# Tarseus/eam-rl4co

Measured on AMD Instinct MI355X. Metric: env-steps/sec (batch x num_loc / s), AttentionModel construction rollout, higher is better.
Workload: dtype f32; 1 GPU; TSP num_loc=100 batch=1024/GPU AM greedy rollout (encoder + cache + decode loop + reward); global_batch=1024, launch=hipGraph replay

## Files before the change

eam_rl4co_amd/csrc/encoder_fused.hip:

```cpp
#include "encoder_fused.hpp"

namespace eamrl {

constexpr int SA = 140;
constexpr int GA = 34;
constexpr int SQ = 66;

struct ALayout {
    float* HB;
    static constexpr int S = SA;
    __device__ float* col(int c) const { return HB + (c & 3) * GA + (c >> 2); }
    __device__ void store4(int row, int q4, float4 v) const
    {
        float* p = HB + row * SA + q4;
        p[0] = v.x; p[GA] = v.y; p[2 * GA] = v.z; p[3 * GA] = v.w;
    }
    __device__ float4 load4(int row, int q4) const
    {
        const float* p = HB + row * SA + q4;
        return make_float4(p[0], p[GA], p[2 * GA], p[3 * GA]);
    }
    __device__ void mirror(int, int, float) const {}
};

#ifdef EAMRL_STAMPS
__device__ unsigned long long g_enc_stamps[24];
#define ESTAMP(i) do { const unsigned long long now_ = __builtin_readcyclecounter(); st_acc[i] += now_ - st_t; st_t = now_; } while (0)
#else
#define ESTAMP(i) do { } while (0)
#endif

__device__ __forceinline__ f32x4 mfma4(float a, float b, f32x4 c) { return __builtin_amdgcn_mfma_f32_16x16x4f32(a, b, c, 0, 0, 0); }

typedef float f32x2v __attribute__((ext_vector_type(2)));
__device__ __forceinline__ float2 lds_read_b64(const float* p)
{
    typedef const volatile __attribute__((address_space(3))) f32x2v* lds_ptr;
    const f32x2v v = *(lds_ptr)(p);
    return make_float2(v.x, v.y);
}

__device__ __forceinline__ float4 global_load_b128(const float* p)
{
    typedef const __attribute__((address_space(1))) f32x4* global_ptr;
    const f32x4 v = *(global_ptr)(p);
    return make_float4(v[0], v[1], v[2], v[3]);
}

template <int CT>
__device__ __forceinline__ void load_b0(float4 (&b0)[CT], const float* const (&wp)[CT])
{
#pragma unroll
    for (int ct = 0; ct < CT; ++ct) b0[ct] = global_load_b128(wp[ct]);
}

template <int RTW, int S>
__device__ __forceinline__ void load_a0(float2 (&a0)[RTW][2], const float* arow, int nrt)
{
#pragma unroll
    for (int rt = 0; rt < RTW; ++rt)
        if (rt < nrt) {
            a0[rt][0] = lds_read_b64(arow + rt * 16 * S);
            a0[rt][1] = lds_read_b64(arow + rt * 16 * S + 2);
        }
}

template <int RTW, int CT, int S, bool SWAP, int NRT, int NU>
__device__ __forceinline__ void gemm_pass_n(f32x4 (&acc)[RTW][CT], const float* arow, const float* const (&wp)[CT],
                                            const float4 (&b0)[CT], const float2 (&a0)[RTW][2])
{
    float4 b[2][CT];
    float2 a[2][NRT][2];
#pragma unroll
    for (int ct = 0; ct < CT; ++ct) b[0][ct] = b0[ct];
#pragma unroll
    for (int rt = 0; rt < NRT; ++rt) { a[0][rt][0] = a0[rt][0]; a[0][rt][1] = a0[rt][1]; }
#pragma unroll
    for (int u = 0; u < NU; ++u) {
        const int c = u & 1, n = c ^ 1;
        __builtin_amdgcn_sched_barrier(0);
        if (u + 1 < NU) {
#pragma unroll
            for (int ct = 0; ct < CT; ++ct) b[n][ct] = global_load_b128(wp[ct] + (u + 1) * 256);
#pragma unroll
            for (int rt = 0; rt < NRT; ++rt) {
                a[n][rt][0] = lds_read_b64(arow + rt * 16 * S + 4 * (u + 1));
                a[n][rt][1] = lds_read_b64(arow + rt * 16 * S + 4 * (u + 1) + 2);
            }
        }
#pragma unroll
        for (int rt = 0; rt < NRT; ++rt) {
#pragma unroll
            for (int ct = 0; ct < CT; ++ct)
                acc[rt][ct] = SWAP ? mfma4(b[c][ct].x, a[c][rt][0].x, acc[rt][ct]) : mfma4(a[c][rt][0].x, b[c][ct].x, acc[rt][ct]);
#pragma unroll
            for (int ct = 0; ct < CT; ++ct)
                acc[rt][ct] = SWAP ? mfma4(b[c][ct].y, a[c][rt][0].y, acc[rt][ct]) : mfma4(a[c][rt][0].y, b[c][ct].y, acc[rt][ct]);
#pragma unroll
            for (int ct = 0; ct < CT; ++ct)
                acc[rt][ct] = SWAP ? mfma4(b[c][ct].z, a[c][rt][1].x, acc[rt][ct]) : mfma4(a[c][rt][1].x, b[c][ct].z, acc[rt][ct]);
#pragma unroll
            for (int ct = 0; ct < CT; ++ct)
                acc[rt][ct] = SWAP ? mfma4(b[c][ct].w, a[c][rt][1].y, acc[rt][ct]) : mfma4(a[c][rt][1].y, b[c][ct].w, acc[rt][ct]);
        }
        if (u + 1 < NU) {
            __builtin_amdgcn_sched_group_barrier(0x20, CT, 0);
#pragma unroll
            for (int i = 0; i < 2 * NRT; ++i) {
                __builtin_amdgcn_sched_group_barrier(0x8, 2, 0);
                __builtin_amdgcn_sched_group_barrier(0x100, 1, 0);
            }
            __builtin_amdgcn_sched_group_barrier(0x8, 4 * NRT * (CT - 1), 0);
        }
    }
    __builtin_amdgcn_sched_barrier(0);
}

template <int RTW, int CT, int S, int NU, bool SWAP = false, int NLOW = RTW>
__device__ __forceinline__ void gemm_pass(f32x4 (&acc)[RTW][CT], const float* arow, int nrt, const float* const (&wp)[CT],
                                          const float4 (&b0)[CT], const float2 (&a0)[RTW][2])
{
    if (NLOW == RTW || nrt == RTW) gemm_pass_n<RTW, CT, S, SWAP, RTW, NU>(acc, arow, wp, b0, a0);
    else gemm_pass_n<RTW, CT, S, SWAP, NLOW, NU>(acc, arow, wp, b0, a0);
}

template <int RTW>
__device__ __forceinline__ void residual_norm_store(const f32x4 (&acc)[RTW][2], float* HB, int row0, int nrt, int cw, int j, int G,
                                                    int norm, const float* cst )
{
    asm volatile("" : "+v"(j), "+v"(G));
#pragma unroll
    for (int ct = 0; ct < 2; ++ct) {
        const int c = 32 * cw + 16 * ct + j;
        const float sc = cst[c], sh = cst[FE + c];
        float* col = HB + (c & 3) * GA + (c >> 2);
#pragma unroll
        for (int rt = 0; rt < RTW; ++rt)
            if (rt < nrt) {
#pragma unroll
                for (int r = 0; r < 4; ++r) {
                    float* p = col + (row0 + 16 * rt + 4 * G + r) * SA;
                    float v = *p + acc[rt][ct][r];
                    if (norm == EAMRL_NORM_BATCH_EVAL) v = fma_(v, sc, sh);
                    *p = v;
                }
            }
    }
}

template <int RTT>
__global__ __launch_bounds__(512, 2) void k_encoder_fused(FusedArgs a)
{
    constexpr int RTA = (RTT + 1) / 2;
    constexpr int RTW = RTA;
    constexpr int ROWS = 16 * RTT;
    constexpr int SV = ROWS + 4;
    extern __shared__ __attribute__((aligned(16))) float lds[];
    float* HB = lds;
    float* QA = HB + ROWS * SA;
    float* KB = QA + ROWS * SQ;
    float* VT = KB + ROWS * SQ;
    float* HID = QA;
    float* CST = VT + 64 * SV;
    static_assert(ROWS * SA <= 2 * ROWS * SQ + 64 * SV, "HID must fit QA | KB | VT");
    const ALayout L{HB};

    const int tid = threadIdx.x, lane = tid & 63;
    const int wv = __builtin_amdgcn_readfirstlane(tid >> 6);
    const int cw = wv & 3, rw = wv >> 2;
    const int j = lane & 15, G = lane >> 4;
    const int M = a.M;
    const int row0 = rw ? 16 * RTA : 0;
    const int nrt = rw ? RTT - RTA : RTA;
    const int64_t inst = blockIdx.x;
    const float* hrow = HB + (row0 + j) * SA + G * GA;
#ifdef EAMRL_STAMPS
    unsigned long long st_acc[20] = {0, 0, 0, 0, 0, 0, 0, 0, 0, 0, 0, 0, 0, 0, 0, 0, 0, 0, 0, 0}, st_t = __builtin_readcyclecounter();
#endif

    if (a.h_in) load_h<ROWS>(a.h_in, M, L);
    else init_embedding<ROWS>(a.init, M, L);
    __syncthreads();
    ESTAMP(0);

    for (int layer = 0; layer < a.nlayers; ++layer) {
        const eamrl_encoder_layer& Ly = a.L[layer];
        const float* wp1[3];
        float4 b1[3];
        float2 a1[RTW][2];
#pragma unroll
        for (int x = 0; x < 3; ++x) wp1[x] = Ly.Wqkv + ((int64_t)(8 * x + cw) * (FE / 16)) * 256 + lane * 4;
        load_b0<3>(b1, wp1);
        load_a0<RTW, SA>(a1, hrow, nrt);
        for (int i = tid; i < NCST; i += blockDim.x) {
            float v;
            if (i < C_BO) v = Ly.bqkv[i];
            else if (i < C_B1) v = Ly.bo[i - C_BO];
            else if (i < C_B2) v = Ly.b1[i - C_B1];
            else if (i < C_N1) v = Ly.b2[i - C_B2];
            else {
                const bool second = i >= C_N2;
                const int k = (i - (second ? C_N2 : C_N1));
                const int c = k & (FE - 1);
                const float* gam = second ? Ly.n2_gamma : Ly.n1_gamma;
                const float* bet = second ? Ly.n2_beta : Ly.n1_beta;
                if (a.norm == EAMRL_NORM_BATCH_EVAL) {
                    const float* mean = second ? Ly.n2_mean : Ly.n1_mean;
                    const float* var = second ? Ly.n2_var : Ly.n1_var;
                    const float sc = gam[c] / __builtin_sqrtf(var[c] + a.eps);
                    const float ms = mean[c] * sc;
                    v = k < FE ? sc : bet[c] - ms;
                } else {
                    v = k < FE ? gam[c] : bet[c];
                }
            }
            CST[i] = v;
        }
        __syncthreads();
        f32x4 acc_o[RTW][2];
#pragma unroll
        for (int ct = 0; ct < 2; ++ct) {
            const float b = CST[C_BO + 32 * cw + 16 * ct + j];
#pragma unroll
            for (int rt = 0; rt < RTW; ++rt) acc_o[rt][ct] = splat4(b);
        }
        for (int hg = 0; hg < 2; ++hg) {
            const float* wp3[2];
            float4 b3[2];
#pragma unroll
            for (int ct = 0; ct < 2; ++ct)
                wp3[ct] = Ly.Wo + ((int64_t)(2 * cw + ct) * (FE / 16) + 4 * hg) * 256 + lane * 4;
            {
                f32x4 acc[RTW][3];
                const int ctq = 4 * hg + cw;
#pragma unroll
                for (int x = 0; x < 3; ++x) {
                    const float b = CST[C_BQKV + 16 * (8 * x + ctq) + j];
#pragma unroll
                    for (int rt = 0; rt < RTW; ++rt) acc[rt][x] = splat4(b);
                }
                ESTAMP(16);
                gemm_pass<RTW, 3, SA, FE / 16, false, RTT - RTA>(acc, hrow, nrt, wp1, b1, a1);
                ESTAMP(17);
                load_b0<2>(b3, wp3);
                int je = j, Ge = G;
                asm volatile("" : "+v"(je), "+v"(Ge));
                float* qcol = QA + (je & 3) * 16 + 4 * cw + (je >> 2);
                float* kcol = KB + (je & 3) * 16 + 4 * cw + (je >> 2);
                float* vrow = VT + (16 * cw + je) * SV;
#pragma unroll
                for (int rt = 0; rt < RTW; ++rt)
                    if (rt < nrt) {
                        const int rbase = row0 + 16 * rt + 4 * Ge;
#pragma unroll
                        for (int r = 0; r < 4; ++r) {
                            qcol[(rbase + r) * SQ] = acc[rt][0][r] * 0.25f;
                            kcol[(rbase + r) * SQ] = acc[rt][1][r];
                        }
                        *reinterpret_cast<float4*>(vrow + rbase) =
                            make_float4(acc[rt][2][0], acc[rt][2][1], acc[rt][2][2], acc[rt][2][3]);
                    }
            }
            ESTAMP(1);
            __syncthreads();
            ESTAMP(2);
            {
                int jp = j, Gp = G;
                asm volatile("" : "+v"(jp), "+v"(Gp));
                const int pi = 4 * (jp & 3) + (jp >> 2);
                float kf[RTT][4];
#pragma unroll
                for (int kt = 0; kt < RTT; ++kt) {
                    const float* p = KB + (16 * kt + pi) * SQ + Gp * 16 + 4 * cw;
                    const float2 lo = *reinterpret_cast<const float2*>(p), hi = *reinterpret_cast<const float2*>(p + 2);
                    kf[kt][0] = lo.x; kf[kt][1] = lo.y; kf[kt][2] = hi.x; kf[kt][3] = hi.y;
                }
                float vf[4 * RTT];
                const int NT = (M + 3) >> 2;
                constexpr int FULLT = RTT == 7 ? 4 : RTT == 4 ? 2 : 0;
#pragma unroll
                for (int t = 0; t < 4 * RTT; ++t) vf[t] = (t < NT) ? VT[(16 * cw + jp) * SV + 4 * t + Gp] : 0.0f;
                for (int q = 0; q < nrt; ++q) {
                    const int qrow = row0 + 16 * q + jp;
                    const float* qp = QA + qrow * SQ + Gp * 16 + 4 * cw;
                    const float2 qlo = *reinterpret_cast<const float2*>(qp), qhi = *reinterpret_cast<const float2*>(qp + 2);
                    f32x4 s[RTT];
                    float m = -INFINITY;
#pragma unroll
                    for (int kt = 0; kt < RTT; ++kt) s[kt] = mfma4(kf[kt][0], qlo.x, splat4(0.0f));
#pragma unroll
                    for (int kt = 0; kt < RTT; ++kt) s[kt] = mfma4(kf[kt][1], qlo.y, s[kt]);
#pragma unroll
                    for (int kt = 0; kt < RTT; ++kt) s[kt] = mfma4(kf[kt][2], qhi.x, s[kt]);
#pragma unroll
                    for (int kt = 0; kt < RTT; ++kt) s[kt] = mfma4(kf[kt][3], qhi.y, s[kt]);
#pragma unroll
                    for (int kt = 0; kt < RTT; ++kt) {
                        if (kt >= FULLT && 16 * kt + 16 > M) {
#pragma unroll
                            for (int r = 0; r < 4; ++r)
                                if (16 * kt + 4 * r + Gp >= M) s[kt][r] = -INFINITY;
                        }
                        m = vmax5_raw(m, s[kt][0], s[kt][1], s[kt][2], s[kt][3]);
                    }
                    {
                        auto r16 = __builtin_amdgcn_permlane16_swap(__float_as_uint(m), __float_as_uint(m), false, false);
                        m = vmax_raw(__uint_as_float(r16[0]), __uint_as_float(r16[1]));
                        auto r32 = __builtin_amdgcn_permlane32_swap(__float_as_uint(m), __float_as_uint(m), false, false);
                        m = vmax_raw(__uint_as_float(r32[0]), __uint_as_float(r32[1]));
                    }
#pragma unroll
                    for (int kt = 0; kt < RTT; ++kt) {
                        f32x2 e01 = (f32x2){s[kt][0], s[kt][1]} - splat2(m), e23 = (f32x2){s[kt][2], s[kt][3]} - splat2(m);
                        d_expf2_nonpos_x2(e01, e23);
                        s[kt] = (f32x4){e01.x, e01.y, e23.x, e23.y};
                    }
                    float zp = s[0][0];
#pragma unroll
                    for (int t = 1; t < 4 * RTT; ++t) zp = zp + s[t >> 2][t & 3];
                    {
                        auto r16 = __builtin_amdgcn_permlane16_swap(__float_as_uint(zp), __float_as_uint(zp), false, false);
                        zp = __uint_as_float(r16[0]) + __uint_as_float(r16[1]);
                        auto r32 = __builtin_amdgcn_permlane32_swap(__float_as_uint(zp), __float_as_uint(zp), false, false);
                        zp = __uint_as_float(r32[0]) + __uint_as_float(r32[1]);
                    }
                    f32x4 o = splat4(0.0f);
#pragma unroll
                    for (int kt = 0; kt < RTT; ++kt)
                        if (kt < FULLT || 16 * kt < M) {
#pragma unroll
                            for (int r = 0; r < 4; ++r) o = mfma4(vf[4 * kt + r], s[kt][r], o);
                        }
                    float* op = QA + qrow * SQ + 4 * cw + Gp;
#pragma unroll
                    for (int r = 0; r < 4; ++r) op[r * 16] = o[r] / zp;
                }
            }
            ESTAMP(3);
            __syncthreads();
            ESTAMP(4);
            float2 a3[RTW][2];
            load_a0<RTW, SQ>(a3, QA + (row0 + j) * SQ + G * 16, nrt);
            if (hg == 0) {
#pragma unroll
                for (int x = 0; x < 3; ++x) wp1[x] += 4 * (FE / 16) * 256;
                load_b0<3>(b1, wp1);
                load_a0<RTW, SA>(a1, hrow, nrt);
            }
            gemm_pass<RTW, 2, SQ, 4, false, RTT - RTA>(acc_o, QA + (row0 + j) * SQ + G * 16, nrt, wp3, b3, a3);
            ESTAMP(5);
            __syncthreads();
            ESTAMP(6);
        }
        const float* wp4[2];
        float4 b4[2];
        float2 a4[RTW][2];
#pragma unroll
        for (int ct = 0; ct < 2; ++ct) wp4[ct] = Ly.W1 + ((int64_t)(2 * cw + ct) * (FE / 16)) * 256 + lane * 4;
        load_b0<2>(b4, wp4);
        residual_norm_store<RTW>(acc_o, HB, row0, nrt, cw, j, G, a.norm, CST + C_N1);
        __syncthreads();
        if (a.norm == EAMRL_NORM_INSTANCE) {
            instance_norm(L, M, a.eps, CST + C_N1);
            __syncthreads();
        }
        load_a0<RTW, SA>(a4, hrow, nrt);
        ESTAMP(7);
        f32x4 acc_f[RTW][2];
#pragma unroll
        for (int ct = 0; ct < 2; ++ct) {
            const float b = CST[C_B2 + 32 * cw + 16 * ct + j];
#pragma unroll
            for (int rt = 0; rt < RTW; ++rt) acc_f[rt][ct] = splat4(b);
        }
        for (int ch = 0; ch < FF / 128; ++ch) {
            const float* wp5[2];
            float4 b5[2];
#pragma unroll
            for (int ct = 0; ct < 2; ++ct)
                wp5[ct] = Ly.W2 + ((int64_t)(2 * cw + ct) * (FF / 16) + 8 * ch) * 256 + lane * 4;
            {
                f32x4 acc[RTW][2];
#pragma unroll
                for (int ct = 0; ct < 2; ++ct) {
                    const float b = CST[C_B1 + 16 * (8 * ch + 2 * cw + ct) + j];
#pragma unroll
                    for (int rt = 0; rt < RTW; ++rt) acc[rt][ct] = splat4(b);
                }
                ESTAMP(14);
                gemm_pass<RTW, 2, SA, FE / 16, false, RTT - RTA>(acc, hrow, nrt, wp4, b4, a4);
                ESTAMP(15);
                load_b0<2>(b5, wp5);
#pragma unroll
                for (int ct = 0; ct < 2; ++ct) {
                    const int c = 32 * cw + 16 * ct + j;
                    float* col = HID + (c & 3) * GA + (c >> 2);
#pragma unroll
                    for (int rt = 0; rt < RTW; ++rt)
                        if (rt < nrt) {
#pragma unroll
                            for (int r = 0; r < 4; ++r) {
                                const float v = acc[rt][ct][r];
                                col[(row0 + 16 * rt + 4 * G + r) * SA] = !(v > 0.0f) ? 0.0f : v;
                            }
                        }
                }
            }
            ESTAMP(8);
            __syncthreads();
            ESTAMP(9);
            float2 a5[RTW][2];
            load_a0<RTW, SA>(a5, HID + (row0 + j) * SA + G * GA, nrt);
            if (ch + 1 < FF / 128) {
#pragma unroll
                for (int ct = 0; ct < 2; ++ct) wp4[ct] += 8 * (FE / 16) * 256;
                load_b0<2>(b4, wp4);
                load_a0<RTW, SA>(a4, hrow, nrt);
            }
            gemm_pass<RTW, 2, SA, 8, false, RTT - RTA>(acc_f, HID + (row0 + j) * SA + G * GA, nrt, wp5, b5, a5);
            ESTAMP(10);
            __syncthreads();
            ESTAMP(11);
        }
        residual_norm_store<RTW>(acc_f, HB, row0, nrt, cw, j, G, a.norm, CST + C_N2);
        __syncthreads();
        if (a.norm == EAMRL_NORM_INSTANCE) {
            instance_norm(L, M, a.eps, CST + C_N2);
            __syncthreads();
        }
        ESTAMP(12);
    }
    if (a.h_out) store_h(a.h_out, M, L);
    ESTAMP(13);
    if (a.cache.gctx) graph_context(a.cache.Wg, a.cache.gctx, M, L, CST);
    if (a.cache.out) {
        float* STG = QA;
        float* crow = a.cache.out + (inst * (int64_t)M) * a.cache.ld;
        for (int sl = 0; sl <= a.cache.nproj; ++sl) {
            const bool lp = sl == a.cache.nproj;
            f32x4 acc[RTW][2];
            const float* wp[2];
            float4 b0[2];
#pragma unroll
            for (int ct = 0; ct < 2; ++ct)
                wp[ct] = (lp ? a.cache.WoutT : a.cache.Wc + (int64_t)sl * FE * FE) + ((int64_t)(2 * cw + ct) * (FE / 16)) * 256 + lane * 4;
            load_b0<2>(b0, wp);
#pragma unroll
            for (int ct = 0; ct < 2; ++ct)
#pragma unroll
                for (int rt = 0; rt < RTW; ++rt) acc[rt][ct] = splat4(0.0f);
            if (lp) __syncthreads();
            const float* arow = (lp ? STG : HB) + (row0 + j) * SA + G * GA;
            float2 a0[RTW][2];
            load_a0<RTW, SA>(a0, arow, nrt);
            gemm_pass<RTW, 2, SA, FE / 16, true, RTT - RTA>(acc, arow, nrt, wp, b0, a0);
#pragma unroll
            for (int rt = 0; rt < RTW; ++rt)
                if (rt < nrt) {
                    const int node = row0 + 16 * rt + j;
#pragma unroll
                    for (int ct = 0; ct < 2; ++ct) {
                        const int c = 32 * cw + 16 * ct + 4 * G;
                        const f32x4 v = acc[rt][ct];
                        if (node < M)
                            *reinterpret_cast<float4*>(crow + (int64_t)node * a.cache.ld + sl * FE + c) = make_float4(v[0], v[1], v[2], v[3]);
                        if (sl == 2) {
                            float* p = STG + node * SA + (c >> 2);
                            p[0] = v[0]; p[GA] = v[1]; p[2 * GA] = v[2]; p[3 * GA] = v[3];
                        }
                    }
                }
        }
    }
#ifdef EAMRL_STAMPS
    if (lane == 0) {
        for (int i = 0; i < 20; ++i) atomicAdd(&g_enc_stamps[i], st_acc[i]);
        atomicAdd(&g_enc_stamps[20], 1ull);
    }
#endif
}

__global__ void k_pack_mfma_b(const float* __restrict__ W, float* __restrict__ Wp, int N, int K)
{
    const int64_t idx = (int64_t)blockIdx.x * blockDim.x + threadIdx.x;
    if (idx >= (int64_t)N * K) return;
    const int q = (int)(idx & 3), l = (int)((idx >> 2) & 63);
    const int64_t blk = idx >> 8;
    const int u = (int)(blk % (K / 16)), ct = (int)(blk / (K / 16));
    const int j = l & 15, g = l >> 4;
    Wp[idx] = W[(int64_t)(16 * ct + j) * K + 16 * u + 4 * q + g];
}

int launch_pack_mfma_b(const float* W, float* Wp, int N, int K, hipStream_t st)
{
    const int64_t n = (int64_t)N * K;
    hipLaunchKernelGGL(k_pack_mfma_b, dim3((unsigned)((n + 255) / 256)), dim3(256), 0, st, W, Wp, N, K);
    return hipGetLastError() == hipSuccess ? 0 : EAMRL_E_LAUNCH;
}

#ifdef EAMRL_STAMPS
extern "C" __attribute__((visibility("default"))) int eamrl_debug_read_enc_stamps(unsigned long long* out, int reset)
{
    if (hipMemcpyFromSymbol(out, HIP_SYMBOL(g_enc_stamps), sizeof(g_enc_stamps)) != hipSuccess) return -1;
    if (reset) {
        unsigned long long z[24] = {0};
        if (hipMemcpyToSymbol(HIP_SYMBOL(g_enc_stamps), z, sizeof(z)) != hipSuccess) return -1;
    }
    return 0;
}
#endif

bool encoder_fused_supports(int M, int E, int H, int FFdim, int nlayers)
{
    return M >= 1 && M <= 112 && E == FE && H == FH && FFdim == FF && nlayers >= 1 && nlayers <= MAX_FUSED_LAYERS;
}

int launch_encoder_fused(const float* h_in, float* h_out, int64_t B, int M, int nlayers, int norm, float eps,
                         const eamrl_encoder_layer* layers, const eamrl_encoder_cache* cache, const eamrl_encoder_init* init,
                         int dtype, hipStream_t st)
{
    if (B <= 0) return 0;
    FusedArgs a = {};
    a.h_in = init ? nullptr : h_in; a.h_out = h_out; a.M = M; a.nlayers = nlayers; a.norm = norm; a.eps = eps;
    if (cache) {
        a.cache = *cache;
        if (!cache->Wg || !cache->gctx) a.cache.Wg = a.cache.gctx = nullptr;
    }
    if (init) a.init = *init;
    for (int l = 0; l < nlayers; ++l) a.L[l] = layers[l];
    if (dtype != DTYPE_F32) return launch_encoder_fused16(a, B, dtype, st);
    return launch_fused(a, B, st, [](auto rtt) {
        constexpr int RTT = decltype(rtt)::value, ROWS = 16 * RTT;
        return FusedVariant{k_encoder_fused<RTT>, ((size_t)ROWS * SA + 2 * (size_t)ROWS * SQ + 64 * (size_t)(ROWS + 4) + NCST) * sizeof(float)};
    });
}

}
```

eam_rl4co_amd/csrc/encoder_fused.hpp:

```cpp
#pragma once
#include <type_traits>

#include "kernels.hpp"

namespace eamrl {

typedef float f32x4 __attribute__((ext_vector_type(4)));

constexpr int FE = 128;
constexpr int FH = 8;
constexpr int FF = 512;
constexpr int MAX_FUSED_LAYERS = 8;
constexpr int NCST = 9 * FE + FF;
constexpr int C_BQKV = 0, C_BO = 3 * FE, C_B1 = 4 * FE, C_B2 = 4 * FE + FF, C_N1 = 5 * FE + FF, C_N2 = 7 * FE + FF;

struct FusedArgs {
    const float* h_in; float* h_out; int M; int nlayers; int norm; float eps;
    eamrl_encoder_cache cache;
    eamrl_encoder_init init;
    eamrl_encoder_layer L[MAX_FUSED_LAYERS];
};


int launch_encoder_fused16(const FusedArgs& a, int64_t B, int dtype, hipStream_t st);

struct FusedVariant {
    void (*kernel)(FusedArgs);
    size_t lds;
};

template <typename Variant>
int launch_fused(const FusedArgs& a, int64_t B, hipStream_t st, Variant variant)
{
    const FusedVariant v = a.M <= 32 ? variant(std::integral_constant<int, 2>())
                         : a.M <= 64 ? variant(std::integral_constant<int, 4>())
                                     : variant(std::integral_constant<int, 7>());
    if (v.lds > 64 * 1024 &&
        hipFuncSetAttribute(reinterpret_cast<const void*>(v.kernel), hipFuncAttributeMaxDynamicSharedMemorySize, (int)v.lds) !=
            hipSuccess)
        return EAMRL_E_LAUNCH;
    hipLaunchKernelGGL(v.kernel, dim3((unsigned)B), dim3(512), v.lds, st, a);
    return hipGetLastError() == hipSuccess ? 0 : EAMRL_E_LAUNCH;
}


template <int ROWS, typename Lay>
__device__ __forceinline__ void load_h(const float* h_in, int M, const Lay L)
{
    const int tid = threadIdx.x;
    constexpr int NLD = (ROWS * (FE / 4) + 511) / 512;
    const float* src = h_in + (int64_t)blockIdx.x * (int64_t)M * FE;
    float4 v[NLD];
#pragma unroll
    for (int u = 0; u < NLD; ++u) {
        const int idx = tid + u * 512;
        const int row = idx / (FE / 4), q4 = idx % (FE / 4);
        v[u] = make_float4(0.f, 0.f, 0.f, 0.f);
        if (row < M) v[u] = *reinterpret_cast<const float4*>(src + (int64_t)row * FE + 4 * q4);
    }
#pragma unroll
    for (int u = 0; u < NLD; ++u) {
        const int idx = tid + u * 512;
        const int row = idx / (FE / 4), q4 = idx % (FE / 4);
        if (row < ROWS) L.store4(row, q4, v[u]);
    }
}

template <int ROWS, typename Lay>
__device__ __forceinline__ void init_embedding(const eamrl_encoder_init in, int M, const Lay L)
{
    const int tid = threadIdx.x;
    const int64_t inst = blockIdx.x;
    const int q4 = tid % (FE / 4), r0 = tid / (FE / 4);
    const int F = in.F;
    float w[4][8], wd[4][2], bb[4], bdv[4];
#pragma unroll
    for (int c = 0; c < 4; ++c) {
        bb[c] = in.b ? in.b[4 * q4 + c] : 0.0f;
        bdv[c] = (in.depot && in.bd) ? in.bd[4 * q4 + c] : 0.0f;
#pragma unroll
        for (int k = 0; k < 8; ++k) w[c][k] = (k < F) ? in.W[(4 * q4 + c) * F + k] : 0.0f;
#pragma unroll
        for (int k = 0; k < 2; ++k) wd[c][k] = in.depot ? in.Wd[(4 * q4 + c) * 2 + k] : 0.0f;
    }
    const float* fsrc = in.feat + inst * (int64_t)M * F;
    float* iout = in.init_out ? in.init_out + inst * (int64_t)M * FE : nullptr;
    for (int row = r0; row < ROWS; row += 16) {
        float y[4] = {0.f, 0.f, 0.f, 0.f};
        if (row < M) {
            if (in.depot && row == 0) {
                const float x0 = in.depot[inst * in.depot_ld], x1 = in.depot[inst * in.depot_ld + 1];
#pragma unroll
                for (int c = 0; c < 4; ++c) y[c] = fma_(x1, wd[c][1], fma_(x0, wd[c][0], bdv[c]));
            } else {
                float x[8];
#pragma unroll
                for (int k = 0; k < 8; ++k) x[k] = (k < F) ? fsrc[(int64_t)row * F + k] : 0.0f;
#pragma unroll
                for (int c = 0; c < 4; ++c) {
                    float acc = bb[c];
#pragma unroll
                    for (int k = 0; k < 8; ++k)
                        if (k < F) acc = fma_(x[k], w[c][k], acc);
                    y[c] = acc;
                }
            }
            if (iout) *reinterpret_cast<float4*>(iout + (int64_t)row * FE + 4 * q4) = make_float4(y[0], y[1], y[2], y[3]);
        }
        L.store4(row, q4, make_float4(y[0], y[1], y[2], y[3]));
    }
}

template <typename Lay>
__device__ __forceinline__ void instance_norm(const Lay L, int M, float eps, const float* cst )
{
    const int c = threadIdx.x;
    if (c < FE) {
        float* col = L.col(c);
        float s = 0.0f;
        for (int n = 0; n < M; ++n) s = s + col[n * Lay::S];
        const float mean = s / (float)M;
        float v = 0.0f;
        for (int n = 0; n < M; ++n) { const float d = col[n * Lay::S] - mean; v = fma_(d, d, v); }
        const float inv = 1.0f / __builtin_sqrtf(v / (float)M + eps);
        const float g = cst[c], bt = cst[FE + c];
        for (int n = 0; n < M; ++n) {
            const float y = fma_((col[n * Lay::S] - mean) * inv, g, bt);
            col[n * Lay::S] = y;
            L.mirror(n, c, y);
        }
    }
}

template <typename Lay>
__device__ __forceinline__ void store_h(float* h_out, int M, const Lay L)
{
    float* dst = h_out + (int64_t)blockIdx.x * (int64_t)M * FE;
    for (int idx = threadIdx.x; idx < M * (FE / 4); idx += blockDim.x) {
        const int row = idx / (FE / 4), q4 = idx % (FE / 4);
        *reinterpret_cast<float4*>(dst + (int64_t)row * FE + 4 * q4) = L.load4(row, q4);
    }
}

template <typename Lay>
__device__ __forceinline__ void graph_context(const float* Wg, float* gctx, int M, const Lay L, float* MEAN)
{
    const int tid = threadIdx.x;
    if (tid < FE) {
        const float* col = L.col(tid);
        float s = 0.0f;
        for (int n = 0; n < M; ++n) s = s + col[n * Lay::S];
        MEAN[tid] = s / (float)M;
    }
    __syncthreads();
    if (tid < FE) {
        const float4* w = reinterpret_cast<const float4*>(Wg + (int64_t)tid * FE);
        float acc = 0.0f;
#pragma unroll 8
        for (int k4 = 0; k4 < FE / 4; ++k4) {
            const float4 wv4 = w[k4];
            acc = fma_(MEAN[4 * k4 + 0], wv4.x, acc);
            acc = fma_(MEAN[4 * k4 + 1], wv4.y, acc);
            acc = fma_(MEAN[4 * k4 + 2], wv4.z, acc);
            acc = fma_(MEAN[4 * k4 + 3], wv4.w, acc);
        }
        gctx[(int64_t)blockIdx.x * FE + tid] = acc;
    }
}

}
```

Baseline: 50.18 million env-steps/s.

## Prefetch next-layer constants and weights, and unroll init embedding loads

Loads of the per-layer bias and norm constants and the first Wqkv weight fragment are now issued for the next layer before the residual norm, so the global-memory latency overlaps with the current layer's work. Each thread holds its constant values in registers and writes them to LDS with a fixed wave-to-slot mapping. The cache-projection weight loads are likewise prefetched one slice ahead. The init embedding is templated on the feature count with branchless, fully unrolled feature loads. Registers held across the layer rise, which may hurt occupancy, and the fixed thread-to-constant mapping assumes a particular block size.

```diff
diff --git a/eam_rl4co_amd/csrc/encoder_fused.hip b/eam_rl4co_amd/csrc/encoder_fused.hip
--- a/eam_rl4co_amd/csrc/encoder_fused.hip
+++ b/eam_rl4co_amd/csrc/encoder_fused.hip
@@ -52,6 +52,58 @@
 {
 #pragma unroll
     for (int ct = 0; ct < CT; ++ct) b0[ct] = global_load_b128(wp[ct]);
+}
+
+__device__ __forceinline__ float global_load_b32(const float* p)
+{
+    typedef const __attribute__((address_space(1))) float* global_ptr;
+    return *(global_ptr)(p);
+}
+
+static_assert(C_BO == 6 * 64 && C_B1 == 512 && C_B2 == 1024 && C_N1 == C_B2 + 2 * 64 && C_N2 == C_N1 + 4 * 64 && NCST == 1536 + 2 * 64,
+              "cst_request / cst_store spell out the CST layout");
+struct CstRaw { float e0, e1, b2, gamma, beta, mean, var; };
+
+__device__ __forceinline__ CstRaw cst_request(const float* bqkv, const float* bo, const float* b1, const float* b2,
+                                              const float* n1_gamma, const float* n1_beta, const float* n1_mean, const float* n1_var,
+                                              const float* n2_gamma, const float* n2_beta, const float* n2_mean, const float* n2_var,
+                                              int norm, int wv, int tid)
+{
+    const int c = tid & (FE - 1);
+    const bool n1 = wv >= 2 && wv < 6, stats = norm == EAMRL_NORM_BATCH_EVAL;
+    const float* gam = n1 ? n1_gamma : n2_gamma;
+    const float* mean = n1 ? n1_mean : n2_mean;
+    const float* var = n1 ? n1_var : n2_var;
+    CstRaw r;
+    r.e0 = global_load_b32((wv < 6 ? bqkv : bo) + (tid - (wv < 6 ? 0 : C_BO)));
+    r.e1 = global_load_b32(b1 + tid);
+    r.b2 = global_load_b32(b2 + c);
+    r.gamma = global_load_b32(gam + c);
+    r.beta = global_load_b32((n1 ? n1_beta : n2_beta) + c);
+    r.mean = global_load_b32((stats ? mean : gam) + c);
+    r.var = global_load_b32((stats ? var : gam) + c);
+    return r;
+}
+
+__device__ __forceinline__ void cst_store(float* CST, const CstRaw r, int norm, float eps, int wv, int tid)
+{
+    const bool shift = wv < 2 || (wv >= 4 && wv < 6);
+    float nv;
+    if (norm == EAMRL_NORM_BATCH_EVAL) {
+        const float sc = r.gamma / __builtin_sqrtf(r.var + eps);
+        const float ms = r.mean * sc;
+        nv = shift ? r.beta - ms : sc;
+    } else {
+        nv = shift ? r.beta : r.gamma;
+    }
+    CST[tid] = r.e0;
+    CST[512 + tid] = r.e1;
+    if (wv < 2) {
+        CST[1024 + tid] = r.b2;
+        CST[1536 + tid] = nv;
+    } else {
+        CST[1024 + tid] = nv;
+    }
 }
 
 template <int RTW, int S>
@@ -175,9 +227,16 @@
     const int64_t inst = blockIdx.x;
     const float* hrow = HB + (row0 + j) * SA + G * GA;
 #ifdef EAMRL_STAMPS
-    unsigned long long st_acc[20] = {0, 0, 0, 0, 0, 0, 0, 0, 0, 0, 0, 0, 0, 0, 0, 0, 0, 0, 0, 0}, st_t = __builtin_readcyclecounter();
+    unsigned long long st_acc[22] = {0, 0, 0, 0, 0, 0, 0, 0, 0, 0, 0, 0, 0, 0, 0, 0, 0, 0, 0, 0, 0, 0}, st_t = __builtin_readcyclecounter();
 #endif
 
+    CstRaw cst = cst_request(a.L[0].bqkv, a.L[0].bo, a.L[0].b1, a.L[0].b2, a.L[0].n1_gamma, a.L[0].n1_beta, a.L[0].n1_mean,
+                             a.L[0].n1_var, a.L[0].n2_gamma, a.L[0].n2_beta, a.L[0].n2_mean, a.L[0].n2_var, a.norm, wv, tid);
+    const float* wp1[3];
+    float4 b1[3];
+#pragma unroll
+    for (int x = 0; x < 3; ++x) wp1[x] = a.L[0].Wqkv + ((int64_t)(8 * x + cw) * (FE / 16)) * 256 + lane * 4;
+    load_b0<3>(b1, wp1);
     if (a.h_in) load_h<ROWS>(a.h_in, M, L);
     else init_embedding<ROWS>(a.init, M, L);
     __syncthreads();
@@ -185,38 +244,11 @@
 
     for (int layer = 0; layer < a.nlayers; ++layer) {
         const eamrl_encoder_layer& Ly = a.L[layer];
-        const float* wp1[3];
-        float4 b1[3];
         float2 a1[RTW][2];
-#pragma unroll
-        for (int x = 0; x < 3; ++x) wp1[x] = Ly.Wqkv + ((int64_t)(8 * x + cw) * (FE / 16)) * 256 + lane * 4;
-        load_b0<3>(b1, wp1);
         load_a0<RTW, SA>(a1, hrow, nrt);
-        for (int i = tid; i < NCST; i += blockDim.x) {
-            float v;
-            if (i < C_BO) v = Ly.bqkv[i];
-            else if (i < C_B1) v = Ly.bo[i - C_BO];
-            else if (i < C_B2) v = Ly.b1[i - C_B1];
-            else if (i < C_N1) v = Ly.b2[i - C_B2];
-            else {
-                const bool second = i >= C_N2;
-                const int k = (i - (second ? C_N2 : C_N1));
-                const int c = k & (FE - 1);
-                const float* gam = second ? Ly.n2_gamma : Ly.n1_gamma;
-                const float* bet = second ? Ly.n2_beta : Ly.n1_beta;
-                if (a.norm == EAMRL_NORM_BATCH_EVAL) {
-                    const float* mean = second ? Ly.n2_mean : Ly.n1_mean;
-                    const float* var = second ? Ly.n2_var : Ly.n1_var;
-                    const float sc = gam[c] / __builtin_sqrtf(var[c] + a.eps);
-                    const float ms = mean[c] * sc;
-                    v = k < FE ? sc : bet[c] - ms;
-                } else {
-                    v = k < FE ? gam[c] : bet[c];
-                }
-            }
-            CST[i] = v;
-        }
+        cst_store(CST, cst, a.norm, a.eps, wv, tid);
         __syncthreads();
+        ESTAMP(18);
         f32x4 acc_o[RTW][2];
 #pragma unroll
         for (int ct = 0; ct < 2; ++ct) {
@@ -422,6 +454,14 @@
             __syncthreads();
             ESTAMP(11);
         }
+        {
+            const eamrl_encoder_layer& Ln = a.L[layer + 1 < a.nlayers ? layer + 1 : layer];
+            cst = cst_request(Ln.bqkv, Ln.bo, Ln.b1, Ln.b2, Ln.n1_gamma, Ln.n1_beta, Ln.n1_mean, Ln.n1_var, Ln.n2_gamma, Ln.n2_beta,
+                              Ln.n2_mean, Ln.n2_var, a.norm, wv, tid);
+#pragma unroll
+            for (int x = 0; x < 3; ++x) wp1[x] = Ln.Wqkv + ((int64_t)(8 * x + cw) * (FE / 16)) * 256 + lane * 4;
+            load_b0<3>(b1, wp1);
+        }
         residual_norm_store<RTW>(acc_f, HB, row0, nrt, cw, j, G, a.norm, CST + C_N2);
         __syncthreads();
         if (a.norm == EAMRL_NORM_INSTANCE) {
@@ -432,19 +472,22 @@
     }
     if (a.h_out) store_h(a.h_out, M, L);
     ESTAMP(13);
+    const float* wpc[2];
+    float4 bc[2];
+    {
+        const float* w0 = !a.cache.out ? a.L[0].Wqkv : a.cache.nproj == 0 ? a.cache.WoutT : a.cache.Wc;
+#pragma unroll
+        for (int ct = 0; ct < 2; ++ct) wpc[ct] = w0 + ((int64_t)(2 * cw + ct) * (FE / 16)) * 256 + lane * 4;
+        load_b0<2>(bc, wpc);
+    }
     if (a.cache.gctx) graph_context(a.cache.Wg, a.cache.gctx, M, L, CST);
+    ESTAMP(19);
     if (a.cache.out) {
         float* STG = QA;
         float* crow = a.cache.out + (inst * (int64_t)M) * a.cache.ld;
         for (int sl = 0; sl <= a.cache.nproj; ++sl) {
             const bool lp = sl == a.cache.nproj;
             f32x4 acc[RTW][2];
-            const float* wp[2];
-            float4 b0[2];
-#pragma unroll
-            for (int ct = 0; ct < 2; ++ct)
-                wp[ct] = (lp ? a.cache.WoutT : a.cache.Wc + (int64_t)sl * FE * FE) + ((int64_t)(2 * cw + ct) * (FE / 16)) * 256 + lane * 4;
-            load_b0<2>(b0, wp);
 #pragma unroll
             for (int ct = 0; ct < 2; ++ct)
 #pragma unroll
@@ -453,7 +496,15 @@
             const float* arow = (lp ? STG : HB) + (row0 + j) * SA + G * GA;
             float2 a0[RTW][2];
             load_a0<RTW, SA>(a0, arow, nrt);
-            gemm_pass<RTW, 2, SA, FE / 16, true, RTT - RTA>(acc, arow, nrt, wp, b0, a0);
+            gemm_pass<RTW, 2, SA, FE / 16, true, RTT - RTA>(acc, arow, nrt, wpc, bc, a0);
+            {
+                const int sn = lp ? sl : sl + 1;
+#pragma unroll
+                for (int ct = 0; ct < 2; ++ct)
+                    wpc[ct] = (sn == a.cache.nproj ? a.cache.WoutT : a.cache.Wc + (int64_t)sn * FE * FE) +
+                              ((int64_t)(2 * cw + ct) * (FE / 16)) * 256 + lane * 4;
+                load_b0<2>(bc, wpc);
+            }
 #pragma unroll
             for (int rt = 0; rt < RTW; ++rt)
                 if (rt < nrt) {
@@ -472,9 +523,11 @@
                 }
         }
     }
+    ESTAMP(21);
 #ifdef EAMRL_STAMPS
     if (lane == 0) {
-        for (int i = 0; i < 20; ++i) atomicAdd(&g_enc_stamps[i], st_acc[i]);
+        for (int i = 0; i < 22; ++i)
+            if (i != 20) atomicAdd(&g_enc_stamps[i], st_acc[i]);
         atomicAdd(&g_enc_stamps[20], 1ull);
     }
 #endif
diff --git a/eam_rl4co_amd/csrc/encoder_fused.hpp b/eam_rl4co_amd/csrc/encoder_fused.hpp
--- a/eam_rl4co_amd/csrc/encoder_fused.hpp
+++ b/eam_rl4co_amd/csrc/encoder_fused.hpp
@@ -66,49 +66,72 @@
     }
 }
 
-template <int ROWS, typename Lay>
-__device__ __forceinline__ void init_embedding(const eamrl_encoder_init in, int M, const Lay L)
+template <int ROWS, int KM, typename Lay>
+__device__ __forceinline__ void init_embedding_f(const eamrl_encoder_init in, int M, const Lay L)
 {
+    constexpr int NT = ROWS / 16;
     const int tid = threadIdx.x;
     const int64_t inst = blockIdx.x;
     const int q4 = tid % (FE / 4), r0 = tid / (FE / 4);
     const int F = in.F;
-    float w[4][8], wd[4][2], bb[4], bdv[4];
+    const bool has_depot = in.depot != nullptr;
+    const float* bp = in.b ? in.b : in.W;
+    const float* bdp = (has_depot && in.bd) ? in.bd : in.W;
+    const float* wdp = has_depot ? in.Wd : in.W;
+    const float* dp = has_depot ? in.depot + inst * in.depot_ld : in.W;
+    const int bm = in.b ? 1 : 0, bdm = (has_depot && in.bd) ? 1 : 0, dm = has_depot ? 1 : 0;
+    float w[4][KM], wd[4][2], bb[4], bdv[4], x[NT][KM];
 #pragma unroll
     for (int c = 0; c < 4; ++c) {
-        bb[c] = in.b ? in.b[4 * q4 + c] : 0.0f;
-        bdv[c] = (in.depot && in.bd) ? in.bd[4 * q4 + c] : 0.0f;
+        bb[c] = bp[(4 * q4 + c) * bm];
+        bdv[c] = bdp[(4 * q4 + c) * bdm];
 #pragma unroll
-        for (int k = 0; k < 8; ++k) w[c][k] = (k < F) ? in.W[(4 * q4 + c) * F + k] : 0.0f;
+        for (int k = 0; k < KM; ++k) w[c][k] = in.W[(4 * q4 + c) * F + (k < F ? k : F - 1)];
 #pragma unroll
-        for (int k = 0; k < 2; ++k) wd[c][k] = in.depot ? in.Wd[(4 * q4 + c) * 2 + k] : 0.0f;
+        for (int k = 0; k < 2; ++k) wd[c][k] = wdp[((4 * q4 + c) * 2 + k) * dm];
     }
+    const float x0 = dp[0], x1 = dp[dm];
     const float* fsrc = in.feat + inst * (int64_t)M * F;
-    float* iout = in.init_out ? in.init_out + inst * (int64_t)M * FE : nullptr;
-    for (int row = r0; row < ROWS; row += 16) {
-        float y[4] = {0.f, 0.f, 0.f, 0.f};
-        if (row < M) {
-            if (in.depot && row == 0) {
-                const float x0 = in.depot[inst * in.depot_ld], x1 = in.depot[inst * in.depot_ld + 1];
 #pragma unroll
-                for (int c = 0; c < 4; ++c) y[c] = fma_(x1, wd[c][1], fma_(x0, wd[c][0], bdv[c]));
-            } else {
-                float x[8];
+    for (int t = 0; t < NT; ++t) {
+        const int row = r0 + 16 * t;
+        const float* fr = fsrc + (int64_t)(row < M ? row : M - 1) * F;
 #pragma unroll
-                for (int k = 0; k < 8; ++k) x[k] = (k < F) ? fsrc[(int64_t)row * F + k] : 0.0f;
+        for (int k = 0; k < KM; ++k) x[t][k] = fr[k < F ? k : F - 1];
+    }
+    __builtin_amdgcn_sched_barrier(0);
+    float y[NT][4];
 #pragma unroll
-                for (int c = 0; c < 4; ++c) {
-                    float acc = bb[c];
+    for (int t = 0; t < NT; ++t) {
+        const int row = r0 + 16 * t;
+        const bool drow = has_depot && row == 0;
 #pragma unroll
-                    for (int k = 0; k < 8; ++k)
-                        if (k < F) acc = fma_(x[k], w[c][k], acc);
-                    y[c] = acc;
-                }
-            }
-            if (iout) *reinterpret_cast<float4*>(iout + (int64_t)row * FE + 4 * q4) = make_float4(y[0], y[1], y[2], y[3]);
+        for (int c = 0; c < 4; ++c) {
+            float acc = bm ? bb[c] : 0.0f;
+#pragma unroll
+            for (int k = 0; k < KM; ++k) acc = (k < F) ? fma_(x[t][k], w[c][k], acc) : acc;
+            const float yd = fma_(x1, wd[c][1], fma_(x0, wd[c][0], bdm ? bdv[c] : 0.0f));
+            y[t][c] = row < M ? (drow ? yd : acc) : 0.0f;
         }
-        L.store4(row, q4, make_float4(y[0], y[1], y[2], y[3]));
     }
+#pragma unroll
+    for (int t = 0; t < NT; ++t) L.store4(r0 + 16 * t, q4, make_float4(y[t][0], y[t][1], y[t][2], y[t][3]));
+    if (in.init_out) {
+        float* iout = in.init_out + inst * (int64_t)M * FE;
+#pragma unroll
+        for (int t = 0; t < NT; ++t) {
+            const int row = r0 + 16 * t;
+            if (row < M) *reinterpret_cast<float4*>(iout + (int64_t)row * FE + 4 * q4) = make_float4(y[t][0], y[t][1], y[t][2], y[t][3]);
+        }
+    }
+}
+
+template <int ROWS, typename Lay>
+__device__ __forceinline__ void init_embedding(const eamrl_encoder_init in, int M, const Lay L)
+{
+    if (in.F <= 2) init_embedding_f<ROWS, 2>(in, M, L);
+    else if (in.F <= 4) init_embedding_f<ROWS, 4>(in, M, L);
+    else init_embedding_f<ROWS, 8>(in, M, L);
 }
 
 template <typename Lay>
```

New measurement: 50.90 million env-steps/s, median of 6. +1.4%, better.
